# NVlabs/sionna

Hardware: AMD Instinct MI355X
Metric: codeword-decodes/sec (n=8448, BP iters=20) (higher is better)
Workload: dtype f32

## Files before the change

sionna_amd/csrc/ldpc5g_jit_gen.cpp:

```cpp
#include "ldpc5g_jit.h"

#include <cstdarg>
#include <functional>

#include "ldpc5g.h"
#include "jit_text.h"

namespace samd {

static bool jit_class1(const samd_ldpc5g* h) {
  if (!h || !h->jit_plan || h->jit_plan->general || !h->ms.g_ok) return false;
  const int z = h->z;
  if (z % 128 != 0 || h->k % 64 != 0 || h->n % 64 != 0) return false;
  if (h->m_int > 0 && (h->n % h->m_int != 0 || (h->n / h->m_int) % 64 != 0)) return false;
  if ((size_t)h->jit_plan->edges * z * 4 > 160 * 1024) return false;
  return true;
}

bool jit_geometry(const samd_ldpc5g* h, bool phi, JitGeometry* out) {
  if (!h || !h->jit_plan) return false;
  const JitPlan& P = *h->jit_plan;
  const int z = h->z;
  if (z < 2 || P.edges <= 0 || P.ncu <= 0) return false;
  if (h->m_int > 0 && h->n % h->m_int != 0) return false;
  for (int r = 0; r < P.ncu; ++r)
    if (P.row_deg[r] < 2 || P.row_deg[r] > 19) return false;
  for (int c = 0; c < P.nbu; ++c)
    if (P.col_edges[c].size() > 30) return false;
  const size_t budget = 160 * 1024;
  double best = -1.0;
  JitGeometry g;
  for (int px = 0; px < 2; ++px) {
    if (!px && (z & 1)) continue;
    const int H = px ? z : z / 2;
    for (int wgs : {1, 2, 4}) {
      const int nw = 16 / wgs;
      for (int G = 1; G <= 64; ++G) {
        const int lanes = G * H, chunks = (lanes + 63) / 64;
        const size_t lds = (size_t)P.edges * lanes * 8 + (phi ? 1024 : 0);
        if (lds * wgs > budget || chunks > 16) break;
        const double eff = (double)lanes / (64.0 * chunks);
        const double fill = std::min(1.0, (double)(P.ncu * chunks) / (2.0 * nw));
        const double score = eff * fill + 1e-3 * std::min(1.0, (double)(G * (px ? 2 : 1) * wgs) / 64.0) - 2e-3 * (wgs - 1) + (px ? 5e-4 : 0.0);
        if (score > best) {
          best = score;
          g.G = G; g.pairx = px; g.H = H; g.P = lanes; g.chunks = chunks; g.blk = 8 * lanes; g.nw = nw; g.wgs = wgs;
        }
      }
    }
  }
  if (best < 0.0 && !phi && !(z & 1)) {
    const int H = z / 2, chunks = (H + 63) / 64;
    const int e_max = (int)(budget / ((size_t)H * 8));
    int r0 = P.ncu;
    while (r0 > 0 && (int)(P.row_off[r0 - 1] / (4 * z)) + P.row_deg[r0 - 1] > e_max) --r0;
    const int e_lds = r0 < P.ncu ? (int)(P.row_off[r0] / (4 * z)) : P.edges;
    if (r0 >= 4 && r0 < P.ncu && (P.edges - e_lds) * 10 <= P.edges * 3 && chunks <= 16) {
      best = 0.0;
      g.G = 1; g.pairx = 0; g.H = H; g.P = H; g.chunks = chunks; g.blk = 8 * H; g.nw = 16; g.wgs = 1;
      g.spill_row = r0; g.e_lds = e_lds; g.ws_bytes = (size_t)(P.edges - e_lds) * g.blk;
    }
  }
  if (best < 0.0) return false;
  if (g.spill_row < 0) g.e_lds = P.edges;
  if (out) *out = g;
  return true;
}

int jit_class(const samd_ldpc5g* h, bool phi) {
  if (!h || !h->jit_plan) return 0;
  if (jit_class1(h)) return 1;
  return jit_geometry(h, phi, nullptr) ? 2 : 0;
}

bool jit_eligible(const samd_ldpc5g* h) { return jit_class(h, false) != 0; }

void build_jit_plan_general(samd_ldpc5g* h, const std::vector<std::vector<std::pair<int, int>>>& by_row) {
  if (h->jit_plan) return;
  const int z = h->z, ncu = (h->n_cn + z - 1) / z, nbu = (h->n_vn + z - 1) / z;
  JitPlan* plan = new JitPlan();
  plan->general = 1;
  plan->z = z; plan->ncu = ncu; plan->nbu = nbu;
  plan->row_off.resize(ncu); plan->row_deg.resize(ncu); plan->fused_col.assign(ncu, -1);
  plan->col_edges.resize(nbu); plan->col_fused.assign(nbu, 0);
  int edges = 0;
  for (int r = 0; r < ncu; ++r) {
    const int d = (int)by_row[r].size();
    plan->row_off[r] = edges * z * 4;
    plan->row_deg[r] = d;
    for (int i = 0; i < d; ++i) {
      const int c = by_row[r][i].first, sft = by_row[r][i].second;
      if (c >= nbu) { delete plan; return; }
      plan->col_edges[c].push_back({(edges + i) * z * 4, 4 * sft});
    }
    edges += d;
  }
  plan->edges = edges;
  for (int r = 0; r < ncu; ++r) {
    const int d = (int)by_row[r].size();
    if (d < 2) continue;
    const int c = by_row[r][d - 1].first, sft = by_row[r][d - 1].second;
    if (plan->col_edges[c].size() == 1 && sft == 0) { plan->fused_col[r] = c; plan->col_fused[c] = 1; }
  }
  if (h->n_cn % z) { plan->prune_row = ncu - 1; plan->prune_z0 = h->n_cn - (ncu - 1) * z; }
  h->jit_plan = plan;
}

namespace {

struct Src {
  std::string s;
  void f(const char* fmt, ...) __attribute__((format(printf, 2, 3))) {
    char buf[1024];
    va_list ap;
    va_start(ap, fmt);
    const int n = vsnprintf(buf, sizeof(buf), fmt, ap);
    va_end(ap);
    if (n > 0) s.append(buf, std::min((size_t)n, sizeof(buf) - 1));
  }
};

struct Chunk {
  enum Kind { LOAD, ZERO, FILLER } kind = ZERO;
  unsigned in_off = 0;
  unsigned out_off = 0xFFFFFFFFu;
  bool out_strided = false;
};

Chunk classify(const samd_ldpc5g* h, int c, int qq, int return_infobits) {
  Chunk r;
  const int z = h->z, v0 = c * z + 64 * qq, fill = h->k_ldpc - h->k;
  int u;
  if (v0 < h->k) u = v0;
  else if (v0 < h->k_ldpc) { r.kind = Chunk::FILLER; return r; }
  else u = v0 - fill;
  if (return_infobits && v0 < h->k) r.out_off = 4u * (unsigned)v0;
  const int t0 = u - 2 * z;
  if (t0 < 0 || t0 >= h->n) return r;
  int o0 = t0;
  if (h->m_int > 0) {
    const int q = h->n / h->m_int;
    o0 = (t0 / q) + (t0 % q) * h->m_int;
  }
  r.kind = Chunk::LOAD;
  r.in_off = 4u * (unsigned)o0;
  if (!return_infobits) { r.out_off = 4u * (unsigned)o0; r.out_strided = true; }
  return r;
}

}

namespace {
struct Sched { std::vector<std::vector<JitItem>> cn, vn; };

struct ItemCost { int cn_slope, cn_ovh, cn_fused, vn_slope, vn_ovh, valu_cn_slope, valu_cn_ovh, valu_cn_fused; };
constexpr ItemCost kCostMinSum = {10, 60, 6, 8, 10, 27, 54, 22};
constexpr ItemCost kCostPhi = {100, 100, 3, 8, 10, 330, 80, 20};
constexpr int kValuVnSlope = 17, kValuVnOvh = 16;

void lpt_assign(std::vector<std::pair<int, JitItem>>& items, int nw, bool rotate, std::vector<std::vector<JitItem>>* out,
                const std::function<int(const JitItem&)>& simd_cost = nullptr) {
  std::stable_sort(items.begin(), items.end(), [](const auto& a, const auto& b) { return a.first > b.first; });
  std::vector<std::vector<std::pair<int, JitItem>>> per(nw);
  std::vector<long> load(nw, 0);
  for (auto& it : items) {
    int w = 0;
    for (int q = 1; q < nw; ++q)
      if (load[q] < load[w]) w = q;
    per[w].push_back(it);
    load[w] += it.first;
  }
  for (int round = 0; round < 64; ++round) {
    const int wm = (int)(std::max_element(load.begin(), load.end()) - load.begin());
    long best = load[wm];
    int bi = -1, bw = -1, bj = -1;
    for (size_t i = 0; i < per[wm].size(); ++i)
      for (int w = 0; w < nw; ++w) {
        if (w == wm) continue;
        const long ci = per[wm][i].first;
        const long m0 = std::max(load[wm] - ci, load[w] + ci);
        if (m0 < best) { best = m0; bi = (int)i; bw = w; bj = -1; }
        for (size_t j = 0; j < per[w].size(); ++j) {
          const long cj = per[w][j].first;
          const long m1 = std::max(load[wm] - ci + cj, load[w] + ci - cj);
          if (cj < ci && m1 < best) { best = m1; bi = (int)i; bw = w; bj = (int)j; }
        }
      }
    if (bi < 0) break;
    const auto a = per[wm][bi];
    if (bj < 0) {
      per[wm].erase(per[wm].begin() + bi);
      per[bw].push_back(a);
      load[wm] -= a.first; load[bw] += a.first;
    } else {
      const auto b = per[bw][bj];
      per[wm][bi] = b; per[bw][bj] = a;
      load[wm] += b.first - a.first; load[bw] += a.first - b.first;
    }
  }
  if (simd_cost && nw >= 8 && nw % 4 == 0) {
    auto simd_load = [&](int q) {
      long t = 0;
      for (int w = q; w < nw; w += 4)
        for (auto& it : per[w]) t += simd_cost(it.second);
      return t;
    };
    const long cap = *std::max_element(load.begin(), load.end());
    for (int round = 0; round < 256; ++round) {
      long sl[4];
      for (int q = 0; q < 4; ++q) sl[q] = simd_load(q);
      const int qm = (int)(std::max_element(sl, sl + 4) - sl);
      long best = sl[qm];
      int bw = -1, bi = -1, cw = -1, cj = -1;
      for (int w = qm; w < nw; w += 4)
        for (size_t i = 0; i < per[w].size(); ++i)
          for (int v = 0; v < nw; ++v) {
            if (v % 4 == qm) continue;
            for (size_t j = 0; j < per[v].size(); ++j) {
              const long ai = simd_cost(per[w][i].second), aj = simd_cost(per[v][j].second);
              if (aj >= ai) continue;
              const long lw = load[w] - per[w][i].first + per[v][j].first, lv = load[v] + per[w][i].first - per[v][j].first;
              if (lw > cap || lv > cap) continue;
              const long m = std::max(sl[qm] - ai + aj, sl[v % 4] + ai - aj);
              if (m < best) { best = m; bw = w; bi = (int)i; cw = v; cj = (int)j; }
            }
          }
      if (bw < 0) break;
      std::swap(per[bw][bi], per[cw][cj]);
      load[bw] += per[bw][bi].first - per[cw][cj].first;
      load[cw] += per[cw][cj].first - per[bw][bi].first;
    }
  }
  for (int w = 0; w < nw; ++w)
    std::stable_sort(per[w].begin(), per[w].end(), [](const auto& a, const auto& b) { return a.first > b.first; });
  const long longest = std::max<long>(1, *std::max_element(load.begin(), load.end()));
  out->assign(nw, {});
  for (int w = 0; w < nw; ++w) {
    if (rotate && per[w].size() > 1) std::rotate(per[w].begin(), per[w].begin() + ((w >> 2) % per[w].size()), per[w].end());
    long rem = load[w];
    for (auto& it : per[w]) {
      JitItem ji = it.second;
      ji.prio = (int)std::max<long>(0, std::min<long>(3, (4 * rem + longest - 1) / longest - 1));
      rem -= it.first;
      (*out)[w].push_back(ji);
    }
  }
}

Sched make_schedule(const samd_ldpc5g* h, bool phi) {
  const JitPlan& P = *h->jit_plan;
  const bool interleaved = h->z == 128;
  Sched s;
  if (!interleaved && !phi) {
    s.cn = P.cn; s.vn = P.vn;
    std::reverse(s.vn.begin(), s.vn.end());
    return s;
  }
  const ItemCost& k = phi ? kCostPhi : kCostMinSum;
  const int cn_pair_max = (phi && !interleaved) ? 12 : 32, vn_pair_max = interleaved ? 30 : 12;
  const int nw = (int)P.cn.size();
  const int chunks = h->z / 64;
  std::vector<std::pair<int, JitItem>> ci, vi;
  for (int r = 0; r < P.ncu; ++r)
    for (int q = 0; q + 1 < chunks; q += 2) {
      const int cost = k.cn_slope * P.row_deg[r] + k.cn_ovh + (P.fused_col[r] >= 0 ? k.cn_fused : 0);
      if (P.row_deg[r] <= cn_pair_max) ci.push_back({cost, JitItem{r, q, 2, 0}});
      else { ci.push_back({cost / 2, JitItem{r, q, 1, 0}}); ci.push_back({cost / 2, JitItem{r, q + 1, 1, 0}}); }
    }
  for (int c = 0; c < P.nbu; ++c) {
    if (P.col_fused[c] || P.col_edges[c].empty()) continue;
    const int d = (int)P.col_edges[c].size();
    for (int q = 0; q + 1 < chunks; q += 2) {
      if (d <= vn_pair_max) vi.push_back({k.vn_slope * d + k.vn_ovh, JitItem{c, q, 2, 0}});
      else {
        vi.push_back({k.vn_slope * d / 2 + k.vn_ovh, JitItem{c, q, 1, 0}});
        vi.push_back({k.vn_slope * d / 2 + k.vn_ovh, JitItem{c, q + 1, 1, 0}});
      }
    }
  }
  const std::function<int(const JitItem&)> ccost = [&P, &k](const JitItem& it) {
    return (k.valu_cn_slope * P.row_deg[it.idx] + k.valu_cn_ovh + (P.fused_col[it.idx] >= 0 ? k.valu_cn_fused : 0)) * it.nch / 2;
  };
  const std::function<int(const JitItem&)> vcost = [&P](const JitItem& it) {
    return (kValuVnSlope * (int)P.col_edges[it.idx].size() + kValuVnOvh) * it.nch / 2;
  };
  lpt_assign(ci, nw, !interleaved, &s.cn, ccost);
  lpt_assign(vi, nw, !interleaved, &s.vn, vcost);
  if (!interleaved) std::reverse(s.vn.begin(), s.vn.end());
  return s;
}
}

static constexpr unsigned kPhiTabBytes = 512u;

static void emit_phi_defines(Src& o) {
  o.f("#define JIT_RULE_PHI 1\n#define JIT_PHI_TAB 0u\n#define JIT_PHI_TAB_ROWS \\\n");
  std::string rows = kJitPhiTabRows;
  const size_t pos = rows.find("*/");
  if (pos != std::string::npos) rows = rows.substr(pos + 2);
  for (char ch : rows) {
    if (ch == '\n') o.s += " \\\n";
    else o.s += ch;
  }
  o.s += "\n";
}

namespace {
enum class Meta { Head, Image, Entry };
void emit_meta(Src& o, const JitProgram& p, Meta which) {
  if (which == Meta::Head) o.f("// JIT_WAVES %d\n", p.waves);
  if (which == Meta::Head && p.wgs > 0) o.f("// JIT_GROUP %d\n// JIT_WGS %d\n// JIT_WS_BYTES %zu\n", p.group, p.wgs, p.ws_bytes);
  if (which == Meta::Image) o.f("// JIT_IMG_BYTES %u\n// JIT_IMG_MSG0 %u\n", p.img_bytes, p.img_msg0);
  if (which == Meta::Entry) o.f("\n// JIT_ENTRY %s\n", p.entry.c_str());
}

const char* const kArgs = "const float* llr_in, float* out, int batch, int num_iter, float llr_max, float offset, int hard_out, float* ws, "
                          "const float* st_in, float* st_out";

struct Emitter {
  const samd_ldpc5g* const h;
  const JitPlan& P;
  const int rib;
  const JitVariant var;
  const bool with_ops, phi;
  const int offset0, z;
  const unsigned msg0;
  const char* bar = "jit_barrier";
  bool ok = false;
  Sched S;
  JitProgram prog;
  Src o;
  int w = 0;
  std::vector<JitItem> cn, vn;

  Emitter(const samd_ldpc5g* h_, int rib_, JitRule rule, bool with_ops_, JitVariant var_)
      : h(h_), P(*h_->jit_plan), rib(rib_), var(var_), with_ops(with_ops_), phi(rule == JitRule::BoxplusPhi),
        offset0(rule == JitRule::MinSum ? 1 : 0), z(h_->z), msg0(phi ? kPhiTabBytes : 0u) {}

  const char* abl4() const { return (var.abl & 4) ? "// " : ""; }
  void begin_wave(int w_) {
    w = w_; cn = S.cn[w]; vn = S.vn[w];
    o.f("\nJIT_DEV void jit_wave_%d(%s) {\n", w, kArgs);
  }
  int vn_deg(size_t j) const { return (int)P.col_edges[vn[j].idx].size(); }
  static std::string numbered(const char* pre, size_t j) { return pre + std::to_string(j); }
  void vb_pair(const char* name, size_t j, const char* mid) {
    const int d = vn_deg(j);
    o.f("      const U32 %s[%d] = {", name, d);
    for (int i = 0; i < d; ++i) o.f("%sva%zu%s_%d", i ? ", " : "", j, mid, i);
    o.f("}; const M64 %s_m[%d] = {", name, d);
    for (int i = 0; i < d; ++i) o.f("%svm%zu_%d", i ? ", " : "", j, i);
    o.f("};\n");
  }
  void state_in_begin(int movers, bool moves = true) {
    if (!var.state) return;
    if (moves) o.f("    if (st_in) { JIT_KEEP_BRANCH(); jit_copy_g2l(st_in + (size_t)b * %uu, %uu, %uu, %d, %d); } else {\n", prog.img_bytes / 4,
                   msg0, prog.img_bytes, w, movers);
    else o.f("    if (st_in) { JIT_KEEP_BRANCH(); } else {\n");
  }
  void state_in_end() { if (var.state) o.f("    }\n"); }
  void state_out(int movers, bool moves = true) {
    if (!var.state) return;
    if (moves) o.f("    if (st_out) { JIT_KEEP_BRANCH(); %s(); jit_copy_l2g(st_out + (size_t)b * %uu, %uu, %uu, %d, %d); %s(); }\n", bar,
                   prog.img_bytes / 4, msg0, prog.img_bytes, w, movers, bar);
    else o.f("    if (st_out) { JIT_KEEP_BRANCH(); %s(); %s(); }\n", bar, bar);
  }
  template <class CnItem, class VnItem>
  void phases(CnItem cn_item, VnItem vn_item) {
    o.f("      {\n");
    for (size_t j = 0; j < cn.size(); ++j) cn_item(j);
    o.f("      }\n      %s%s();\n", abl4(), bar);
    o.f("      {\n");
    for (size_t j = 0; j < vn.size(); ++j) vn_item(j);
    o.f("      }\n");
  }
  template <class CnItem, class VnItem>
  void loop_with_last(CnItem cn_item, VnItem vn_item) {
    o.f("#pragma unroll 1\n    for (int it = 0; it < num_iter; ++it) {\n      const bool last = it == num_iter - 1;\n      (void)last;\n");
    phases(cn_item, vn_item);
    o.f("      %sif (!last) %s();\n    }\n", abl4(), bar);
  }
  void entry() {
    if (!with_ops) return;
    emit_meta(o, prog, Meta::Entry);
    o.f("extern \"C\" __global__ __launch_bounds__(%d) void %s(%s) {\n", 64 * prog.waves, prog.entry.c_str(), kArgs);
    o.f("  __shared__ float jit_smem[JIT_LDS_FLOATS];\n");
    o.f("  if ((unsigned)(unsigned long)(jit_lds_f32*)jit_smem != 0u) __builtin_trap();\n");
    o.f("  switch (jit_wave()) {\n");
    for (int v = 0; v < prog.waves; ++v)
      o.f("    case %d: jit_wave_%d(llr_in, out, batch, num_iter, llr_max, offset, hard_out, ws, st_in, st_out); break;\n", v, v);
    o.f("    default: break;\n  }\n}\n");
  }
};

struct GeneralEmitter : Emitter {
  JitGeometry g;
  bool px = false, spill = false, wave_part = false;
  int H = 0, nw = 0, chunks = 0, nw_full = 0, cwg = 0, nout = 0;
  struct Need { std::string raw[2], in[2], out[2], cw[2]; int q; };
  std::vector<Need> needs;
  std::vector<int> cn_need;

  GeneralEmitter(const samd_ldpc5g* h_, int rib_, JitRule rule, bool with_ops_, JitVariant var_) : Emitter(h_, rib_, rule, with_ops_, var_) {
    if (!jit_geometry(h, phi, &g)) return;
    H = g.H; nw = g.nw; chunks = g.chunks; px = g.pairx != 0; spill = g.spill_row >= 0;
    cwg = px ? 2 * g.G : g.G; nout = rib ? h->k : h->n;
    schedule();
    if (var.state && (spill || nw_full == 0)) return;
    if (spill) bar = "jit_barrier_g";
    Src entry;
    entry.f("samd_ldpc5g_jit_%s%s_bg%dz%dk%dn%d", phi ? "phi" : offset0 ? "ms" : "oms", var.state ? "_st" : "", h->bg, z, h->k, h->n);
    prog.entry = entry.s;
    prog.waves = nw; prog.group = cwg; prog.wgs = g.wgs; prog.ws_bytes = g.ws_bytes;
    prog.img_bytes = (unsigned)(g.e_lds * g.blk); prog.img_msg0 = msg0; prog.layout_b = true;
    ok = true;
  }
  void schedule() {
    const ItemCost& k = phi ? kCostPhi : kCostMinSum;
    const bool partial = (g.P % 64) != 0;
    int nw_part = 0;
    if (partial) nw_part = chunks == 1 ? nw : std::max(1, std::min(nw - 1, (nw + chunks / 2) / chunks));
    nw_full = nw - nw_part;
    std::vector<std::pair<int, JitItem>> ci[2], vi[2];
    for (int r = 0; r < P.ncu; ++r)
      for (int q = 0; q < chunks; ++q)
        ci[partial && q == chunks - 1].push_back({k.cn_slope * P.row_deg[r] + k.cn_ovh + (P.fused_col[r] >= 0 ? k.cn_fused : 0), JitItem{r, q, 2, 0}});
    for (int c = 0; c < P.nbu; ++c) {
      if (P.col_fused[c] || P.col_edges[c].empty()) continue;
      for (int q = 0; q < chunks; ++q)
        vi[partial && q == chunks - 1].push_back({k.vn_slope * (int)P.col_edges[c].size() + k.vn_ovh, JitItem{c, q, 2, 0}});
    }
    Sched sa, sb;
    if (nw_full > 0) { lpt_assign(ci[0], nw_full, true, &sa.cn); lpt_assign(vi[0], nw_full, true, &sa.vn); }
    if (nw_part > 0) { lpt_assign(ci[1], nw_part, true, &sb.cn); lpt_assign(vi[1], nw_part, true, &sb.vn); }
    std::reverse(sa.vn.begin(), sa.vn.end()); std::reverse(sb.vn.begin(), sb.vn.end());
    S.cn = sa.cn; S.cn.insert(S.cn.end(), sb.cn.begin(), sb.cn.end());
    S.vn = sa.vn; S.vn.insert(S.vn.end(), sb.vn.begin(), sb.vn.end());
  }
  int edge_index(int32_t first) const { return (int)(first / (4 * z)); }
  bool e_sp(int e) const { return e >= g.e_lds; }
  unsigned e_off(int e) const {
    return e >= g.e_lds ? (unsigned)((e - g.e_lds) * g.blk) : msg0 + (unsigned)(e * g.blk);
  }
  unsigned cn_base(const JitItem& it) const { return e_off(edge_index(P.row_off[it.idx])) + 512u * (unsigned)it.q; }
  bool cn_sp(const JitItem& it) const { return spill && it.idx >= g.spill_row; }
  unsigned vn_spm(const JitItem& it) const {
    unsigned mk = 0u;
    const auto& ed = P.col_edges[it.idx];
    for (size_t i = 0; i < ed.size(); ++i)
      if (e_sp(edge_index(ed[i].first))) mk |= 1u << i;
    return mk;
  }

  void header() {
    emit_meta(o, prog, Meta::Head);
    o.f("#define JIT_NWAVES %d\n#define JIT_WS_FLOATS %zu\n", nw, g.ws_bytes / 4);
    if (spill)
      o.f("// messages beyond LDS: base rows >= %d (%d of %d edges) in the workgroup's row of the workspace (L2)\n", g.spill_row,
          P.edges - g.e_lds, P.edges);
    o.f("// specialised 5G LDPC decoder (any lifting size): BG%d Z=%d k=%d n=%d m_int=%d pruned=%d return_infobits=%d %s\n", h->bg, z,
        h->k, h->n, h->m_int, h->nb_pruned, rib, phi ? "boxplus-phi" : offset0 ? "min-sum" : "offset-min-sum");
    o.f("// geometry: %d codewords per workgroup (%s), %d lanes in %d chunks, %d bytes per edge block, %d workgroup(s) per CU\n", cwg,
        px ? "a slot = copy z of two codewords" : "a slot = copies z, z + Z/2 of one codeword", g.P, chunks, g.blk, g.wgs);
    o.f("#define JIT_OFFSET0 %d\n#define JIT_GENERAL 1\n#define JIT_LAYOUT_B 1\n", offset0 ? 1 : 0);
    const unsigned lds_msg = ((msg0 + (unsigned)(g.e_lds * g.blk)) + 511u) & ~511u;
    if (phi) emit_phi_defines(o);
    if (var.state) emit_meta(o, prog, Meta::Image);
    const int stride = h->m_int > 0 ? h->m_int : 1;
    o.f("#define JIT_Z4 %uu\n#define JIT_Z %d\n#define JIT_H %d\n#define JIT_G %d\n#define JIT_P %d\n", (unsigned)g.blk, z, H, cwg, g.P);
    o.f("#define JIT_K %d\n#define JIT_KLDPC %d\n#define JIT_FILLERS %d\n#define JIT_N %d\n#define JIT_NOUT %d\n#define JIT_M %uu\n"
        "#define JIT_Q %d\n#define JIT_RIB %d\n#define JIT_LDS_FLOATS %u\n",
        h->k, h->k_ldpc, h->k_ldpc - h->k, h->n, nout, (unsigned)stride, h->n / stride, rib ? 1 : 0, lds_msg / 4);
    if (var.abl) o.f("#define JIT_ABL %d\n", var.abl);
    if (with_ops) o.s += kJitOps;
    o.s += kJitTemplates;
  }
  void prologue() {
    wave_part = w >= nw_full;
    o.f("  const U32 ln = jit_lane();\n  const U32 l8 = u_shl(ln, 3);\n  (void)offset; (void)hard_out; (void)st_in; (void)st_out;\n");
    o.f("  float* wsw = ws + (size_t)JIT_BLOCK * JIT_WS_FLOATS;\n  (void)wsw;\n");
    if (phi && w == 0) o.f("  jit_phi_stage(u_shl(ln, 2));\n");
    std::vector<char> used(chunks, 0);
    for (auto& it : cn) used[it.q] = 1;
    for (auto& it : vn) used[it.q] = 1;
    for (int q = 0; q < chunks; ++q)
      if (used[q])
        o.f("  const U32 p%d = ln + %uu; const M64 act%d = u_lt(p%d, %uu); const U32 g%d = u_div(p%d, %uu); const U32 z%d = p%d - g%d * %uu;\n",
            q, 64u * q, q, q, (unsigned)g.P, q, q, (unsigned)H, q, q, q, (unsigned)H);
    if (wave_part) o.f("  JIT_IF(act%d)\n", chunks - 1);
    for (size_t j = 0; j < vn.size(); ++j) {
      const JitItem& it = vn[j];
      const auto& ed = P.col_edges[it.idx];
      for (size_t i = 0; i < ed.size(); ++i) {
        const int sft = ed[i].second / 4, sh = sft % H, hi = (!px && sft >= H) ? 1 : 0;
        Src swap;
        if (px) swap.f("jit_no_swap()");
        else swap.f("jit_vn_swap_g(z%d, %uu, %s)", it.q, (unsigned)sh, hi ? "true" : "false");
        o.f("  const U32 va%zu_%zu = jit_vn_addr_g(p%d, z%d, %uu, %uu); const M64 vm%zu_%zu = %s;\n", j, i, it.q, it.q, (unsigned)sh,
            e_off(edge_index(ed[i].first)), j, i, swap.s.c_str());
      }
      o.f("  // ^ column %d chunk %d\n", it.idx, it.q);
    }
  }
  void add_need(const char* pre, size_t j, int c, int q) {
    Need nd;
    nd.q = q;
    for (int hh = 0; hh < 2; ++hh) {
      Src r, cwn, a, b;
      if (px) cwn.f("g%d + g%d + %uu", q, q, (unsigned)hh);
      else cwn.f("g%d", q);
      const unsigned node = (unsigned)(px ? c * z : c * z + hh * H);
      r.f("r%s%zu_%d", pre, j, hh);
      a.f("jit_in_off(u_here(z%d) + %uu, %s, act%d)", q, node, cwn.s.c_str(), q);
      b.f("jit_out_off(u_here(z%d) + %uu, %s, act%d, %s)", q, node, cwn.s.c_str(), q, a.s.c_str());
      nd.raw[hh] = r.s; nd.in[hh] = a.s; nd.out[hh] = b.s; nd.cw[hh] = cwn.s;
    }
    needs.push_back(nd);
  }
  void channel() {
    needs.clear();
    cn_need.assign(cn.size(), -1);
    for (size_t j = 0; j < vn.size(); ++j) add_need("v", j, vn[j].idx, vn[j].q);
    for (size_t j = 0; j < cn.size(); ++j)
      if (P.fused_col[cn[j].idx] >= 0) { cn_need[j] = (int)needs.size(); add_need("c", j, P.fused_col[cn[j].idx], cn[j].q); }
    o.f("  const int ngroups = (batch + %d) / %d;\n", cwg - 1, cwg);
    const unsigned row_in = (unsigned)(cwg * h->n), row_out = (unsigned)(cwg * nout);
    o.f("#pragma unroll 1\n  for (int b = JIT_BLOCK; b < ngroups; b += JIT_GRID) {\n");
    o.f("    float* orow = out + (size_t)b * %uu;\n    const int rem = batch - b * %d;\n    (void)orow; (void)rem;\n", row_out, cwg);
    o.f("    const float* rows = llr_in + (size_t)b * %uu;\n", row_in);
    for (auto& nd : needs)
      for (int hh = 0; hh < 2; ++hh)
        o.f("    F32 %s = jit_ld_raw(rows, %s, %s, rem, llr_max);\n", nd.raw[hh].c_str(), nd.in[hh].c_str(), nd.cw[hh].c_str());
    for (size_t j = 0; j < vn.size(); ++j)
      o.f("    const F32 lv%zu[2] = {jit_chan(%s, llr_max), jit_chan(%s, llr_max)};\n", j, needs[j].raw[0].c_str(), needs[j].raw[1].c_str());
    for (size_t j = 0; j < cn.size(); ++j)
      if (cn_need[j] >= 0)
        o.f("    const F32 lc%zu[2] = {jit_chan(%s, llr_max), jit_chan(%s, llr_max)};\n", j, needs[cn_need[j]].raw[0].c_str(),
            needs[cn_need[j]].raw[1].c_str());
  }
  void init() {
    state_in_begin(nw_full, !wave_part);
    for (size_t j = 0; j < vn.size(); ++j) {
      o.f("    {\n");
      vb_pair("vb", j, "");
      o.f("      jit_vnb_init<%d, 0x%xu>(vb, vb_m, lv%zu, wsw);\n    }\n", vn_deg(j), vn_spm(vn[j]), j);
    }
    for (size_t j = 0; j < cn.size(); ++j)
      if (P.fused_col[cn[j].idx] >= 0)
        o.f("    jit_cn_init_fused<%d, 2, %s>(jit_base(l8, %uu), lc%zu, wsw);\n", P.row_deg[cn[j].idx], cn_sp(cn[j]) ? "true" : "false",
            cn_base(cn[j]), j);
    state_in_end();
    o.f("    %s();\n", bar);
  }
  void emit_out(const Need& nd) {
    o.f(" if (last) {");
    for (int hh = 0; hh < 2; ++hh) o.f(" jit_st_out(orow, %s, %s, rem, xo[%d], llr_max, hard_out);", nd.out[hh].c_str(), nd.cw[hh].c_str(), hh);
    o.f(" }");
  }
  void cn_item(size_t j) {
    const JitItem& it = cn[j];
    const int d = P.row_deg[it.idx];
    const bool fuse = P.fused_col[it.idx] >= 0, prune = it.idx == P.prune_row;
    if (phi) o.f("      const U32 ca%zu = jit_base(l8, %uu);\n", j, cn_base(it));
    else o.f("      const U32 ca%zu = jit_base(l8, %uu); F32 cv%zu[%d][2]; jit_cn_load<%d, 2, %s>(cv%zu, ca%zu, wsw);\n", j, cn_base(it), j, d, d,
             cn_sp(it) ? "true" : "false", j, j);
    o.f("      jit_setprio<%d>();\n", it.prio & 3);
    o.f("      { F32 xo[2];");
    if (prune && px) o.f(" const M64 pm[2] = {u_ge(z%d, %uu), u_ge(z%d, %uu)};", it.q, (unsigned)P.prune_z0, it.q, (unsigned)P.prune_z0);
    else if (prune) o.f(" const M64 pm[2] = {u_ge(z%d, %uu), u_ge(z%d + %uu, %uu)};", it.q, (unsigned)P.prune_z0, it.q, (unsigned)H, (unsigned)P.prune_z0);
    else o.f(" const M64 pm[2] = {};");
    if (!fuse) o.f(" const F32 nolf[2] = {};");
    const std::string lf = fuse ? numbered("lc", j) : "nolf";
    if (phi) o.f(" jit_cn_phi_rolled<%s, %s>(ca%zu, %d, %s, llr_max, xo, pm);", fuse ? "true" : "false", prune ? "true" : "false", j, d,
                 lf.c_str());
    else o.f(" jit_cn_update<%d, 2, %s, %s, %s>(cv%zu, ca%zu, %s, llr_max, offset, xo, pm, wsw);", d, fuse ? "true" : "false",
             prune ? "true" : "false", cn_sp(it) ? "true" : "false", j, j, lf.c_str());
    if (fuse) emit_out(needs[cn_need[j]]);
    o.f(" }\n");
  }
  void vn_item(size_t j) {
    const int d = vn_deg(j);
    vb_pair(numbered("vb", j).c_str(), j, "");
    o.f("      F32 vc%zu[%d][2]; jit_vnb_load<%d, 0x%xu>(vc%zu, vb%zu, wsw);\n", j, d, d, vn_spm(vn[j]), j, j);
    o.f("      jit_setprio<%d>();\n", vn[j].prio & 3);
    o.f("      { F32 xo[2]; jit_vnb_update<%d, 0x%xu>(vc%zu, vb%zu, vb%zu_m, lv%zu, llr_max, xo, wsw);", d, vn_spm(vn[j]), j, j, j, j);
    emit_out(needs[j]);
    o.f(" }\n");
  }
  void iterations() { loop_with_last([this](size_t j) { cn_item(j); }, [this](size_t j) { vn_item(j); }); }
  void end_wave() {
    state_out(nw_full, !wave_part);
    o.f("  }\n%s}\n", wave_part ? "  JIT_END\n" : "");
  }
};

struct Class1Emitter : Emitter {
  const int z4, stride;
  const bool lb;
  const bool lean_last;
  const char* const lrow;
  std::vector<int> edge_col;
  std::vector<char> col_last;
  struct Need { std::string name; Chunk ch; };
  std::vector<Need> needs;
  enum Phase { BOTH, INNER, LAST };

  Class1Emitter(const samd_ldpc5g* h_, int rib_, JitRule rule, bool with_ops_, JitVariant var_)
      : Emitter(h_, rib_, rule, with_ops_, var_), z4(4 * z), stride(h_->m_int > 0 ? h_->m_int : 1), lb(z == 128),
        lean_last(!phi && !var.state), lrow(lb ? "l8" : "l4") {
    S = make_schedule(h, phi);
    prog.entry = phi ? (var.state ? "samd_ldpc5g_jit_phi_st" : "samd_ldpc5g_jit_phi") : (var.state ? "samd_ldpc5g_jit_st" : "samd_ldpc5g_jit");
    prog.waves = (int)S.cn.size();
    ok = true;
    prog.img_bytes = (unsigned)(P.edges * z4); prog.img_msg0 = msg0; prog.layout_b = lb;
  }
  void header() {
    emit_meta(o, prog, Meta::Head);
    o.f("#define JIT_NWAVES %d\n", prog.waves);
    o.f("// specialised 5G LDPC decoder: BG%d Z=%d k=%d n=%d m_int=%d pruned=%d return_infobits=%d %s\n", h->bg, z, h->k, h->n,
        h->m_int, h->nb_pruned, rib, offset0 ? "min-sum" : "offset-min-sum");
    o.f("#define JIT_OFFSET0 %d\n", offset0 ? 1 : 0);
    if (phi) emit_phi_defines(o);
    o.f("#define JIT_Z4 %uu\n#define JIT_N %d\n#define JIT_NOUT %d\n#define JIT_M %uu\n#define JIT_LDS_FLOATS %d\n", (unsigned)z4,
        h->n, rib ? h->k : h->n, (unsigned)stride, P.edges * z + (phi ? 128 : 0));
    if (lb) o.f("#define JIT_LAYOUT_B 1\n");
    if (var.abl) o.f("#define JIT_ABL %d\n", var.abl);
    if (var.state) { emit_meta(o, prog, Meta::Image); o.f("// state=1\n"); }
    if (with_ops) o.s += kJitOps;
    o.s += kJitTemplates;
    edge_col.assign(P.edges, 0);
    col_last.assign(P.nbu, 0);
    for (int c = 0; c < P.nbu; ++c) {
      for (auto& ed : P.col_edges[c]) edge_col[ed.first / z4] = c;
      if (P.col_fused[c]) continue;
      for (int qq = 0; qq < z / 64; ++qq)
        if (classify(h, c, qq, rib).out_off != 0xFFFFFFFFu) col_last[c] = 1;
    }
  }
  bool vnb(size_t j) const { return lb && vn[j].nch == 2; }
  void prologue() {
    o.f("  const U32 l4 = jit_lane4();\n  const U32 l4m = l4 * JIT_M;\n  (void)l4m; (void)offset; (void)ws; (void)st_in; (void)st_out;\n");
    if (lb) o.f("  const U32 l8 = l4 + l4;\n  (void)l8;\n");
    if (phi && w == 0) o.f("  jit_phi_stage(l4);\n");
    for (size_t j = 0; j < vn.size(); ++j) {
      const JitItem& it = vn[j];
      const auto& ed = P.col_edges[it.idx];
      const int d = (int)ed.size();
      if (vnb(j)) {
        for (int i = 0; i < d; ++i) {
          const int s4 = ed[i].second % z4;
          const int k8 = (512 - (2 * s4) % 512) % 512, kb = (512 - s4) % 512;
          Src bit;
          if (var.abl & 16) bit.f("l4 & 0u");
          else bit.f("l4 + %uu", (unsigned)kb);
          o.f("  const U32 va%zu_0_%d = jit_vn_addr(l8, %uu, %uu); const M64 vm%zu_%d = u_testbit(%s, 256u);\n", j, i, (unsigned)k8,
              msg0 + (unsigned)ed[i].first, j, i, bit.s.c_str());
        }
      } else if (lb) {
        for (int i = 0; i < d; ++i) {
          const int kk = (((256 * it.q - ed[i].second) % z4) + z4) % z4;
          o.f("  const U32 va%zu_0_%d = jit_vn_addr_b1(l4, %uu, %uu);\n", j, i, (unsigned)kk, msg0 + (unsigned)ed[i].first);
        }
      } else {
        for (int hh = 0; hh < it.nch; ++hh)
          for (int i = 0; i < d; ++i) {
            const int kk = (((256 * (it.q + hh) - ed[i].second) % z4) + z4) % z4;
            o.f("  const U32 va%zu_%d_%d = jit_vn_addr(l4, %uu, %uu);\n", j, hh, i, (unsigned)kk, msg0 + (unsigned)ed[i].first);
          }
      }
      o.f("  // ^ column %d chunk %d\n", it.idx, it.q);
    }
  }
  void add_need(const char* pre, size_t j, int hh, int c, int qq) {
    needs.push_back({numbered(pre, j) + "_" + std::to_string(hh), classify(h, c, qq, rib)});
  }
  std::string chan_expr(const Need& nd) const {
    if (nd.ch.kind == Chunk::LOAD) return "jit_chan(" + nd.name + ", llr_max)";
    if (nd.ch.kind == Chunk::FILLER) return std::string("jit_chan(jit_bcast(-llr_max), llr_max)");
    return std::string("jit_chan(jit_bcast(0.f), llr_max)");
  }
  void channel() {
    needs.clear();
    for (size_t j = 0; j < vn.size(); ++j)
      for (int hh = 0; hh < vn[j].nch; ++hh) add_need("rv", j, hh, vn[j].idx, vn[j].q + hh);
    for (size_t j = 0; j < cn.size(); ++j)
      if (P.fused_col[cn[j].idx] >= 0)
        for (int hh = 0; hh < cn[j].nch; ++hh) add_need("rc", j, hh, P.fused_col[cn[j].idx], cn[j].q + hh);
    o.f("#pragma unroll 1\n  for (int b = JIT_BLOCK; b < batch; b += JIT_GRID) {\n");
    o.f("    float* orow = out + (size_t)b * JIT_NOUT;\n    (void)orow;\n");
    o.f("    const float* row = llr_in + (size_t)b * JIT_N;\n");
    for (auto& nd : needs)
      if (nd.ch.kind == Chunk::LOAD) o.f("    F32 %s = g_ld(row, l4m, %uu);\n", nd.name.c_str(), nd.ch.in_off);
    size_t ni = 0;
    auto values = [&](const char* nm, size_t j, int nch) {
      o.f("    const F32 %s%zu[%d] = {", nm, j, nch);
      for (int hh = 0; hh < nch; ++hh, ++ni) o.f("%s%s", hh ? ", " : "", chan_expr(needs[ni]).c_str());
      o.f("};\n");
    };
    for (size_t j = 0; j < vn.size(); ++j) values("lv", j, vn[j].nch);
    for (size_t j = 0; j < cn.size(); ++j)
      if (P.fused_col[cn[j].idx] >= 0) values("lc", j, cn[j].nch);
  }
  void emit_vb(const char* name, size_t j) {
    const JitItem& it = vn[j];
    const int d = vn_deg(j);
    if (vnb(j)) return vb_pair(name, j, "_0");
    o.f("      const U32 %s[%d][%d] = {", name, d, it.nch);
    for (int i = 0; i < d; ++i) {
      o.f("%s{", i ? ", " : "");
      for (int hh = 0; hh < it.nch; ++hh) o.f("%sva%zu_%d_%d", hh ? ", " : "", j, hh, i);
      o.f("}");
    }
    o.f("};\n");
  }
  unsigned cn_base(const JitItem& it) const { return msg0 + (unsigned)(P.row_off[it.idx] + (lb ? 4 : 256) * it.q); }
  void init() {
    state_in_begin(prog.waves);
    for (size_t j = 0; j < vn.size(); ++j) {
      o.f("    {\n");
      emit_vb("vb", j);
      if (vnb(j)) o.f("      jit_vnb_init<%d>(vb, vb_m, lv%zu);\n    }\n", vn_deg(j), j);
      else o.f("      jit_vn_init<%d, %d>(vb, lv%zu);\n    }\n", vn_deg(j), vn[j].nch, j);
    }
    for (size_t j = 0; j < cn.size(); ++j)
      if (P.fused_col[cn[j].idx] >= 0)
        o.f("    jit_cn_init_fused<%d, %d>(jit_base(%s, %uu), lc%zu);\n", P.row_deg[cn[j].idx], cn[j].nch, lrow, cn_base(cn[j]), j);
    state_in_end();
    o.f("    jit_barrier();\n");
  }
  struct Out { unsigned oc[2] = {0xFFFFFFFFu, 0xFFFFFFFFu}; bool strided = false, any = false; };
  Out out_offs(int c, const JitItem& it) const {
    Out r;
    for (int hh = 0; hh < it.nch; ++hh) {
      const Chunk ch = classify(h, c, it.q + hh, rib);
      r.oc[hh] = ch.out_off;
      if (ch.out_off != 0xFFFFFFFFu) { r.strided = ch.out_strided; r.any = true; }
    }
    return r;
  }
  void emit_out(const Out& t, int nch, Phase ph) {
    if (!t.any || ph == INNER) return;
    o.f(ph == LAST ? "      {" : "      if (last) {");
    for (int hh = 0; hh < nch; ++hh)
      if (t.oc[hh] != 0xFFFFFFFFu)
        o.f(" g_st(orow, u_here(%s), 0x%xu, jit_outval(xo[%d], llr_max, hard_out));", t.strided ? "l4m" : "l4", t.oc[hh], hh);
    o.f(" }\n");
  }
  void cn_item(size_t j, Phase ph) {
    const JitItem& it = cn[j];
    const int fc = P.fused_col[it.idx], d = P.row_deg[it.idx];
    const bool rolled = phi && lb && it.nch == 2;
    if (rolled) o.f("      const U32 ca%zu = jit_base(%s, %uu);\n", j, lrow, cn_base(it));
    else o.f("      const U32 ca%zu = jit_base(%s, %uu); F32 cv%zu[%d][%d]; jit_cn_load<%d, %d>(cv%zu, ca%zu);\n", j, lrow, cn_base(it), j, d,
             it.nch, d, it.nch, j, j);
    const Out t = fc >= 0 ? out_offs(fc, it) : Out();
    o.f("      jit_setprio<%d>();\n", it.prio & 3);
    o.f("      { F32 xo[%d]; const M64 nopm[%d] = {};", it.nch, it.nch);
    const bool fuse = fc >= 0 && (ph != LAST || t.any);
    const std::string lf = fuse ? numbered("lc", j) : "nolf";
    const char *tf = fuse ? "true" : "false", *lfn = lf.c_str();
    if (!fuse) o.f(" const F32 nolf[%d] = {};", it.nch);
    if (rolled) {
      o.f(" jit_cn_phi_rolled<%s, false>(ca%zu, %d, %s, llr_max, xo, nopm);\n", tf, j, d, lfn);
    } else if (phi) {
      o.f(" jit_cn_update_phi<%d, %d, %s>(cv%zu, ca%zu, %s, llr_max, xo, nopm);\n", d, it.nch, tf, j, j, lfn);
    } else if (ph == LAST) {
      unsigned keep = 0u;
      for (int i = 0; i < d; ++i)
        if (col_last[edge_col[P.row_off[it.idx] / z4 + i]]) keep |= 1u << i;
      o.f(" jit_cn_update<%d, %d, %s, false, false, 0x%xu>(cv%zu, ca%zu, %s, llr_max, offset, xo, nopm);\n", d, it.nch, tf, keep, j, j, lfn);
    } else {
      o.f(" jit_cn_update<%d, %d, %s>(cv%zu, ca%zu, %s, llr_max, offset, xo, nopm);\n", d, it.nch, tf, j, j, lfn);
    }
    emit_out(t, it.nch, ph);
    o.f("      }\n");
  }
  void vn_item(size_t j, Phase ph) {
    const JitItem& it = vn[j];
    const int d = vn_deg(j);
    const Out t = out_offs(it.idx, it);
    if (ph == LAST && !t.any) return;
    emit_vb(numbered("vb", j).c_str(), j);
    if (vnb(j)) o.f("      F32 vc%zu[%d][2]; jit_vnb_load<%d>(vc%zu, vb%zu);\n", j, d, d, j, j);
    else o.f("      F32 vc%zu[%d][%d]; jit_vn_load<%d, %d>(vc%zu, vb%zu);\n", j, d, it.nch, d, it.nch, j, j);
    o.f("      jit_setprio<%d>();\n", it.prio & 3);
    o.f("      { F32 xo[%d];", it.nch);
    if (ph == LAST) {
      if (vnb(j)) o.f(" jit_vnb_total<%d>(vc%zu, vb%zu_m, lv%zu, xo);\n", d, j, j, j);
      else o.f(" jit_vn_total<%d, %d>(vc%zu, lv%zu, xo);\n", d, it.nch, j, j);
    } else {
      if (vnb(j)) o.f(" jit_vnb_update<%d>(vc%zu, vb%zu, vb%zu_m, lv%zu, llr_max, xo);\n", d, j, j, j, j);
      else o.f(" jit_vn_update<%d, %d>(vc%zu, vb%zu, lv%zu, llr_max, xo);\n", d, it.nch, j, j, j);
    }
    emit_out(t, it.nch, ph);
    o.f("      }\n");
  }
  void iterations() {
    auto items = [this](Phase ph) { phases([this, ph](size_t j) { cn_item(j, ph); }, [this, ph](size_t j) { vn_item(j, ph); }); };
    if (!lean_last) { loop_with_last([this](size_t j) { cn_item(j, BOTH); }, [this](size_t j) { vn_item(j, BOTH); }); return; }
    o.f("#pragma unroll 1\n    for (int it = 1; it < num_iter; ++it) {\n");
    items(INNER);
    o.f("      %sjit_barrier();\n    }\n", abl4());
    o.f("    if (num_iter > 0) {\n");
    items(LAST);
    o.f("    }\n");
  }
  void end_wave() { state_out(prog.waves); o.f("  }\n}\n"); }
};

}

JitRule jit_rule(int cn_mode) {
  return cn_mode == SAMD_CN_OFFSET_MINSUM ? JitRule::OffsetMinSum : cn_mode == SAMD_CN_MINSUM ? JitRule::MinSum
         : cn_mode == SAMD_CN_BOXPLUS_PHI ? JitRule::BoxplusPhi : JitRule::None;
}

JitProgram jit_generate(const samd_ldpc5g* h, int return_infobits, JitRule rule, bool with_ops, JitVariant var) {
  const int cls = rule == JitRule::None ? 0 : jit_class(h, rule == JitRule::BoxplusPhi);
  auto run = [](auto&& e) {
    if (!e.ok) return JitProgram();
    e.header();
    for (int v = 0; v < e.prog.waves; ++v) {
      e.begin_wave(v);
      e.prologue();
      e.channel();
      e.init();
      e.iterations();
      e.end_wave();
    }
    e.entry();
    e.prog.source = std::move(e.o.s);
    return std::move(e.prog);
  };
  if (cls == 1) return run(Class1Emitter(h, return_infobits, rule, with_ops, var));
  if (cls == 2) return run(GeneralEmitter(h, return_infobits, rule, with_ops, var));
  return JitProgram();
}

int jit_state_layout(const samd_ldpc5g* h, JitRule rule, JitProgram* p, JitGeometry* g) {
  if (!h || !h->jit_plan || rule == JitRule::None) return 0;
  const JitVariant sv{1, 0};
  const int cls = jit_class(h, rule == JitRule::BoxplusPhi);
  if (cls == 1) *p = Class1Emitter(h, 1, rule, false, sv).prog;
  if (cls == 2) {
    const GeneralEmitter e(h, 1, rule, false, sv);
    if (!e.ok) return 0;
    *p = e.prog;
    if (g) *g = e.g;
  }
  return cls;
}

int jit_state_map(const samd_ldpc5g* h, JitRule rule, int32_t* cw, int32_t* cn, int32_t* vn) {
  JitProgram prog;
  JitGeometry g;
  const int cls = jit_state_layout(h, rule, &prog, &g);
  if (!cls) return SAMD_ERR_UNSUPPORTED;
  const int img = (int)(prog.img_bytes / 4);
  const JitPlan& P = *h->jit_plan;
  const int z = h->z;
  for (int q = 0; q < img; ++q) cw[q] = cn[q] = vn[q] = -1;
  std::vector<int> brow(P.edges, -1), bcol(P.edges, -1), bsh(P.edges, 0);
  for (int r = 0; r < P.ncu; ++r)
    for (int i = 0; i < P.row_deg[r]; ++i) brow[P.row_off[r] / (4 * z) + i] = r;
  for (int c = 0; c < P.nbu; ++c)
    for (auto& ed : P.col_edges[c]) {
      const int e = ed.first / (4 * z);
      if (e < 0 || e >= P.edges) return SAMD_ERR_INVALID;
      bcol[e] = c;
      bsh[e] = (ed.second / 4) % z;
    }
  for (int e = 0; e < P.edges; ++e) {
    if (brow[e] < 0 || bcol[e] < 0) return SAMD_ERR_INVALID;
    const int r = brow[e], c = bcol[e], s = bsh[e];
    auto put = [&](int q, int j, int zc) {
      if (r == P.prune_row && zc >= P.prune_z0) return;
      cw[q] = j; cn[q] = r * z + zc; vn[q] = c * z + (zc + s) % z;
    };
    if (cls == 1) {
      for (int zc = 0; zc < z; ++zc) {
        const int f = prog.layout_b ? 2 * (zc & 63) + (zc >> 6) : zc;
        put(e * z + f, 0, zc);
      }
    } else {
      const int bf = g.blk / 4;
      for (int p = 0; p < g.P; ++p) {
        const int gq = p / g.H, zz = p % g.H;
        if (g.pairx) { put(e * bf + 2 * p, 2 * gq, zz); put(e * bf + 2 * p + 1, 2 * gq + 1, zz); }
        else { put(e * bf + 2 * p, gq, zz); put(e * bf + 2 * p + 1, gq, zz + g.H); }
      }
    }
  }
  return SAMD_OK;
}

}
```

Measured before the change: 4.348 million.

## Peel first BP iteration specialized for zero-LLR punctured columns

Adds a specialized first-iteration path to the generated class-1 LDPC kernel. Columns whose channel LLRs are known to be zero (punctured or pruned) start with zero variable-to-check messages, so the first check-node pass only needs to compute the message toward the single zero-column edge of each row. The first variable-node pass for those columns then uses simplified templates that touch only the edges that have real messages. It adds code-generation complexity and only applies when every check row contains a zero column, so it may not be enabled for a given code geometry.

```diff
diff --git a/sionna_amd/csrc/jit/ldpc5g_jit_first.h b/sionna_amd/csrc/jit/ldpc5g_jit_first.h
--- /dev/null
+++ b/sionna_amd/csrc/jit/ldpc5g_jit_first.h
@@ -0,0 +1,78 @@
+
+template <int D, int NCH, bool FUSE, int PE>
+JIT_DEV void jit_cn_first(U32 a0, const F32 (&lf)[NCH], float llr_max, float offset) {
+  F32 v[D][NCH];
+#pragma unroll
+  for (int i = 0; i < D; ++i) {
+    if (i == PE) continue;
+    if (FUSE && i == D - 1) {
+#pragma unroll
+      for (int h = 0; h < NCH; ++h) v[i][h] = lf[h];
+    } else if (JIT_LAYOUT_B && NCH == 2) lds_ld2(a0, (unsigned)i * JIT_Z4, v[i][0], v[i][NCH - 1]);
+    else {
+#pragma unroll
+      for (int h = 0; h < NCH; ++h) v[i][h] = lds_ld(a0, (unsigned)i * JIT_Z4 + JIT_CH * h);
+    }
+  }
+  F32 c2v[NCH];
+#pragma unroll
+  for (int h = 0; h < NCH; ++h) {
+    F32 m = f_abs(v[PE == 0 ? 1 : 0][h]);
+    U32 sx = 0u;
+#pragma unroll
+    for (int k = 0; k < D - 1; ++k) {
+      const int i = k < PE ? k : k + 1, ip = (k - 1) < PE ? k - 1 : k;
+      if (k >= 1) m = f_med3(m, f_abs(v[i][h]), 0.f);
+      if (k & 1) sx = u_xor3(sx, f_bits(v[ip][h]), f_bits(v[i][h]));
+      else if (k == D - 2) sx = sx ^ f_bits(v[i][h]);
+    }
+    const F32 a = JIT_OFFSET0 ? m : f_med3(m - offset, 0.f, llr_max);
+    c2v[h] = u_float(f_bits(a) | (sx & 0x80000000u));
+  }
+  jit_cn_store<NCH>(a0, (unsigned)PE * JIT_Z4, c2v);
+}
+
+template <int D, unsigned HAVE>
+JIT_DEV void jit_vnb_first(const U32 (&a)[D], const M64 (&sw)[D], const F32 (&l)[2], float llr_max) {
+  F32 x0 = 0.f, x1 = 0.f;
+  F32 v0[D], v1[D];
+#pragma unroll
+  for (int i = 0; i < D; ++i) {
+    if (!((HAVE >> i) & 1u)) continue;
+    F32 c0, c1;
+    lds_ld2(a[i], 0u, c0, c1);
+    v0[i] = f_sel(sw[i], c1, c0);
+    v1[i] = f_sel(sw[i], c0, c1);
+    f_pk_add(x0, x1, v0[i], v1[i]);
+  }
+  f_pk_add(x0, x1, l[0], l[1]);
+  const F32 y0 = f_med3(x0, -llr_max, llr_max), y1 = f_med3(x1, -llr_max, llr_max);
+#pragma unroll
+  for (int i = 0; i < D; ++i) {
+    F32 e0 = y0, e1 = y1;
+    if ((HAVE >> i) & 1u) {
+      f_pk_sub(e0, e1, x0, x1, v0[i], v1[i]);
+      e0 = f_med3(e0, -llr_max, llr_max);
+      e1 = f_med3(e1, -llr_max, llr_max);
+    }
+    lds_st2(a[i], 0u, f_sel(sw[i], e1, e0), f_sel(sw[i], e0, e1));
+  }
+}
+template <int D, int NCH, unsigned HAVE>
+JIT_DEV void jit_vn_first(const U32 (&a)[D][NCH], const F32 (&l)[NCH], float llr_max) {
+#pragma unroll
+  for (int h = 0; h < NCH; ++h) {
+    F32 c[D];
+    F32 x = 0.f;
+#pragma unroll
+    for (int i = 0; i < D; ++i) {
+      if (!((HAVE >> i) & 1u)) continue;
+      c[i] = lds_ld(a[i][h], 0u);
+      x = x + c[i];
+    }
+    x = x + l[h];
+    const F32 y = f_med3(x, -llr_max, llr_max);
+#pragma unroll
+    for (int i = 0; i < D; ++i) lds_st(a[i][h], 0u, ((HAVE >> i) & 1u) ? f_med3(x - c[i], -llr_max, llr_max) : y);
+  }
+}
diff --git a/sionna_amd/csrc/ldpc5g_jit_gen.cpp b/sionna_amd/csrc/ldpc5g_jit_gen.cpp
--- a/sionna_amd/csrc/ldpc5g_jit_gen.cpp
+++ b/sionna_amd/csrc/ldpc5g_jit_gen.cpp
@@ -601,6 +601,9 @@
   const char* const lrow;
   std::vector<int> edge_col;
   std::vector<char> col_last;
+  bool lean_first = false;
+  std::vector<char> col_zero;
+  std::vector<int> row_zeros, row_pe, edge_row;
   struct Need { std::string name; Chunk ch; };
   std::vector<Need> needs;
   enum Phase { BOTH, INNER, LAST };
@@ -630,12 +633,26 @@
     o.s += kJitTemplates;
     edge_col.assign(P.edges, 0);
     col_last.assign(P.nbu, 0);
+    col_zero.assign(P.nbu, 1);
     for (int c = 0; c < P.nbu; ++c) {
       for (auto& ed : P.col_edges[c]) edge_col[ed.first / z4] = c;
+      for (int qq = 0; qq < z / 64; ++qq)
+        if (classify(h, c, qq, rib).kind != Chunk::ZERO) col_zero[c] = 0;
       if (P.col_fused[c]) continue;
       for (int qq = 0; qq < z / 64; ++qq)
         if (classify(h, c, qq, rib).out_off != 0xFFFFFFFFu) col_last[c] = 1;
     }
+    row_zeros.assign(P.ncu, 0); row_pe.assign(P.ncu, -1); edge_row.assign(P.edges, 0);
+    lean_first = lean_last && !var.abl;
+    for (int r = 0; r < P.ncu; ++r) {
+      for (int i = 0; i < P.row_deg[r]; ++i) {
+        const int e = P.row_off[r] / z4 + i;
+        edge_row[e] = r;
+        if (col_zero[edge_col[e]]) { ++row_zeros[r]; row_pe[r] = i; }
+      }
+      if (row_zeros[r] == 0 || (P.fused_col[r] >= 0 && col_zero[P.fused_col[r]])) lean_first = false;
+    }
+    if (lean_first) o.s += kJitFirst;
   }
   bool vnb(size_t j) const { return lb && vn[j].nch == 2; }
   void prologue() {
@@ -714,19 +731,58 @@
     o.f("};\n");
   }
   unsigned cn_base(const JitItem& it) const { return msg0 + (unsigned)(P.row_off[it.idx] + (lb ? 4 : 256) * it.q); }
-  void init() {
-    state_in_begin(prog.waves);
+  void init_stores(int zero) {
     for (size_t j = 0; j < vn.size(); ++j) {
+      if (zero >= 0 && (col_zero[vn[j].idx] != 0) != (zero != 0)) continue;
       o.f("    {\n");
       emit_vb("vb", j);
       if (vnb(j)) o.f("      jit_vnb_init<%d>(vb, vb_m, lv%zu);\n    }\n", vn_deg(j), j);
       else o.f("      jit_vn_init<%d, %d>(vb, lv%zu);\n    }\n", vn_deg(j), vn[j].nch, j);
     }
+    if (zero == 1) return;
     for (size_t j = 0; j < cn.size(); ++j)
       if (P.fused_col[cn[j].idx] >= 0)
         o.f("    jit_cn_init_fused<%d, %d>(jit_base(%s, %uu), lc%zu);\n", P.row_deg[cn[j].idx], cn[j].nch, lrow, cn_base(cn[j]), j);
+  }
+  unsigned have_mask(int c) const {
+    unsigned mk = 0u;
+    for (size_t i = 0; i < P.col_edges[c].size(); ++i)
+      if (row_zeros[edge_row[P.col_edges[c][i].first / z4]] == 1) mk |= 1u << i;
+    return mk;
+  }
+  void init() {
+    state_in_begin(prog.waves);
+    init_stores(lean_first ? 0 : -1);
     state_in_end();
-    o.f("    jit_barrier();\n");
+    if (!lean_first) { o.f("    jit_barrier();\n"); return; }
+    bool owner = false;
+    for (size_t j = 0; j < vn.size(); ++j) owner |= col_zero[vn[j].idx] != 0;
+    if (owner) {
+      o.f("    if (num_iter < 2) {\n");
+      init_stores(1);
+      o.f("    }\n");
+    }
+    o.f("    jit_barrier();\n    if (num_iter >= 2) {\n      jit_setprio<0>();\n      {\n");
+    for (size_t j = 0; j < cn.size(); ++j) {
+      const JitItem& it = cn[j];
+      const int r = it.idx;
+      if (row_zeros[r] != 1) continue;
+      const bool fuse = P.fused_col[r] >= 0;
+      o.f("      {");
+      if (!fuse) o.f(" const F32 nolf[%d] = {};", it.nch);
+      o.f(" jit_cn_first<%d, %d, %s, %d>(jit_base(%s, %uu), %s, llr_max, offset); }\n", P.row_deg[r], it.nch, fuse ? "true" : "false",
+          row_pe[r], lrow, cn_base(it), fuse ? numbered("lc", j).c_str() : "nolf");
+    }
+    o.f("      }\n      jit_barrier();\n      {\n");
+    for (size_t j = 0; j < vn.size(); ++j) {
+      if (!col_zero[vn[j].idx]) continue;
+      const int d = vn_deg(j);
+      o.f("      {\n");
+      emit_vb("vb", j);
+      if (vnb(j)) o.f("      jit_vnb_first<%d, 0x%xu>(vb, vb_m, lv%zu, llr_max);\n      }\n", d, have_mask(vn[j].idx), j);
+      else o.f("      jit_vn_first<%d, %d, 0x%xu>(vb, lv%zu, llr_max);\n      }\n", d, vn[j].nch, have_mask(vn[j].idx), j);
+    }
+    o.f("      }\n      jit_barrier();\n    }\n");
   }
   struct Out { unsigned oc[2] = {0xFFFFFFFFu, 0xFFFFFFFFu}; bool strided = false, any = false; };
   Out out_offs(int c, const JitItem& it) const {
@@ -798,12 +854,14 @@
   void iterations() {
     auto items = [this](Phase ph) { phases([this, ph](size_t j) { cn_item(j, ph); }, [this, ph](size_t j) { vn_item(j, ph); }); };
     if (!lean_last) { loop_with_last([this](size_t j) { cn_item(j, BOTH); }, [this](size_t j) { vn_item(j, BOTH); }); return; }
+    if (lean_first) o.f("    const int jit_rest = num_iter >= 2 ? num_iter - 1 : num_iter;\n    {\n    const int num_iter = jit_rest;\n");
     o.f("#pragma unroll 1\n    for (int it = 1; it < num_iter; ++it) {\n");
     items(INNER);
     o.f("      %sjit_barrier();\n    }\n", abl4());
     o.f("    if (num_iter > 0) {\n");
     items(LAST);
     o.f("    }\n");
+    if (lean_first) o.f("    }\n");
   }
   void end_wave() { state_out(prog.waves); o.f("  }\n}\n"); }
 };
```

Measured after the change: 4.417 million (median of 6 runs). +1.6%, better.
